# yjxiong/action-detection

Measured on AMD Instinct MI355X. Metric: proposals/sec (9-seg BNInception SSN fwd+bwd), higher is better.
Workload: dtype f32

## Files before the change

### action-detection_amd/_lib.py

```python
import ctypes
import os
import subprocess
import threading

import torch

_HERE = os.path.dirname(os.path.abspath(__file__))
CSRC = os.path.join(_HERE, "csrc")
LIB_PATH = os.path.join(_HERE, "libssn_hip.so")
SOURCES = ["conv_igemm.hip", "conv_x6.hip", "conv_x6_rect.hip", "conv_wgrad.hip", "conv_wgrad_x6.hip", "elementwise.hip", "bn_train.hip", "frames.hip", "detect.hip", "pool.hip", "stpp.hip", "heads_losses.hip", "conv_pl.hip", "planes_ops.hip", "planes_bn.hip", "wgrad_pl.hip", "tag.hip", "eval.hip", "actionness.hip", "train_step.hip", "flow.hip"]

STPP_MAX_PARTS = 24


class SsnStppTable(ctypes.Structure):
    _fields_ = [("n_parts", ctypes.c_int), ("n_seg", ctypes.c_int),
                ("act_lo", ctypes.c_int), ("act_hi", ctypes.c_int),
                ("lo", ctypes.c_int * STPP_MAX_PARTS), ("hi", ctypes.c_int * STPP_MAX_PARTS),
                ("norm", ctypes.c_int * STPP_MAX_PARTS), ("col", ctypes.c_int * STPP_MAX_PARTS)]


_SIGS = {
    "ssn_conv_bn_relu_fwd": "pppppiiiiliiiliiiiipp",
    "ssn_bn_fold": "pppppfppip",
# ... 179 lines not shown
        for name, sig in _SIGS.items():
            fn = getattr(self.cdll, name)
            fn.restype = ctypes.c_int
            fn.argtypes = [_CT[c] for c in sig]
            self._fn[name] = fn

    def call(self, name, *args):
        rc = self._fn[name](*args)
        if rc != 0:
            raise RuntimeError("%s failed (%d): %s" % (name, rc, self.cdll.ssn_last_error().decode()))

    def wgrad_workspace_bytes(self, n, cin, cout, ho, wo, ksize, tile_cfg=-1):
        return int(self.cdll.ssn_conv_wgrad_workspace_bytes(n, cin, cout, ho, wo, ksize, tile_cfg))


_lock = threading.Lock()
_lib = None
_test_lib = None


def _source_stamp(deps, flags):
    import hashlib
    h = hashlib.sha256(" ".join(flags).encode())
    for d in deps:
        h.update(os.path.basename(d).encode())
        with open(d, "rb") as f:
            h.update(f.read())
    return h.hexdigest()


def build(force=False, verbose=False):
    import fcntl
    srcs = [os.path.join(CSRC, s) for s in SOURCES]
    deps = srcs + [os.path.join(CSRC, h) for h in ("ssn_common.h", "conv_epilogue.h", "conv_x6_kernel.h", "planes.h", "conv_pl_epilogue.inc")]
    flags = ["--offload-arch=gfx950", "-O3", "-std=c++17", "-fPIC"]
    stamp_path = LIB_PATH + ".stamp"
    want = _source_stamp(deps, flags)

    def fresh():
        if not os.path.exists(LIB_PATH) or not os.path.exists(stamp_path):
            return False
        with open(stamp_path) as f:
            return f.read().strip() == want

    if not force and fresh():
        return LIB_PATH
    with open(LIB_PATH + ".lock", "w") as lock:
        fcntl.flock(lock, fcntl.LOCK_EX)
        try:
            if not force and fresh():
                return LIB_PATH
            hipcc = os.environ.get("HIPCC", "/opt/rocm/bin/hipcc")
            objs = []
            procs = []
            headers = deps[len(srcs):]
            for s in srcs:
                o = os.path.join(CSRC, os.path.basename(s) + ".o")
                objs.append(o)
                ostamp = _source_stamp([s] + headers, flags)
                try:
                    with open(o + ".stamp") as f:
                        if not force and os.path.exists(o) and f.read().strip() == ostamp:
                            continue
                except OSError:
                    pass
                cmd = [hipcc] + flags + ["-c", s, "-o", o]
                procs.append((cmd, o, ostamp, subprocess.Popen(cmd, stdout=subprocess.PIPE, stderr=subprocess.STDOUT)))
# ... 41 lines not shown
```

### action-detection_amd/csrc/conv_wgrad.hip

```cpp
#include <type_traits>

#include "ssn_common.h"

namespace {

struct WgradArgs {
    const float* g;
    const float* x;
    float* part;
    int N, Cin, H, W;
    long x_img_stride;
    int M, Ho, Wo;
    long g_img_stride;
    int K;
    int ldp;
    int P;
    int pad;
    int splits, chunks_per_split;
    int n_mtiles, n_ktiles;
    uint32_t g_bytes, x_bytes;
    FastDiv div_hw, div_w, div_tiles, div_kt;
};

constexpr int BP = 32;
constexpr int PITCH = 36;
constexpr uint32_t OOB = 0x80000000u;

__device__ __forceinline__ __amdgpu_buffer_rsrc_t make_rsrc(const void* base, uint32_t bytes) {
    return __builtin_amdgcn_make_buffer_rsrc(const_cast<void*>(base), 0, (int)bytes, 0x00020000);
}

template <int KS, int S, int WM, int WN, int TM, int TN>
__global__ __launch_bounds__(256) void conv_wgrad_kernel(WgradArgs p) {
    constexpr int BM = WM * TM * 32;
    constexpr int BN = WN * TN * 32;
// ... 147 lines not shown
#pragma unroll
                    for (int j = 0; j < TN; ++j)
                        acc[i][j] = __builtin_amdgcn_mfma_f32_32x32x2f32(af[cur][i][s], bf[cur][j][s], acc[i][j], 0, 0, 0);
        }
        if (t + 1 < nch) store_slab(buf ^ 1);
        __syncthreads();
    }

    float* out = p.part + (long)z * p.M * p.ldp;
#pragma unroll
    for (int j = 0; j < TN; ++j) {
        const int kk = kk0 + (wn * TN + j) * 32 + li;
        if (kk >= p.K) continue;
#pragma unroll
        for (int i = 0; i < TM; ++i) {
#pragma unroll
            for (int r = 0; r < 16; ++r) {
                const int m = m0 + (wm * TM + i) * 32 + (r & 3) + 8 * (r >> 2) + 4 * lh;
                if (m < p.M) out[(long)m * p.ldp + kk] = acc[i][j][r];
            }
        }
    }
    if (do_bias) {
#pragma unroll
        for (int i = 0; i < TM; ++i) {
            const float tot = rowsum[i] + __shfl_xor(rowsum[i], 32, 64);
            const int m = m0 + (wm * TM + i) * 32 + li;
            if (lh == 0 && m < p.M) out[(long)m * p.ldp + p.K] = tot;
        }
    }
}

__global__ __launch_bounds__(256) void wgrad_reduce_kernel(const float* part, float* dw, float* db, int M, int K,
                                                           int ldp, int splits, int taps) {
    const long total = (long)M * ldp;
    for (long idx = (long)blockIdx.x * 256 + threadIdx.x; idx < total; idx += (long)gridDim.x * 256) {
        float s = 0.f;
        int z = 0;
        for (; z + 8 <= splits; z += 8) {
            float v[8];
#pragma unroll
            for (int q = 0; q < 8; ++q) v[q] = part[(long)(z + q) * total + idx];
#pragma unroll
            for (int q = 0; q < 8; ++q) s += v[q];
        }
        for (; z < splits; ++z) s += part[(long)z * total + idx];
        const int m = (int)(idx / ldp);
        const int kk = (int)(idx - (long)m * ldp);
        if (kk < K) {
            int col = kk;
            if (taps > 1) {
                const int cin = K / taps, t = kk / cin;
                col = (kk - t * cin) * taps + t;
            }
            dw[(long)m * K + col] = s;
        } else if (db) {
            db[m] = s;
        }
    }
}

constexpr int RM_MAX = 48;
struct ReduceTable {
    const float* part[RM_MAX];
    float* dw[RM_MAX];
    float* db[RM_MAX];
    int M[RM_MAX], K[RM_MAX], splits[RM_MAX], taps[RM_MAX];
    int blk0[RM_MAX + 1];
    int count;
};
__global__ __launch_bounds__(256) void wgrad_reduce_multi_kernel(ReduceTable t) {
    int ti = 0;
    while (ti + 1 < t.count && (int)blockIdx.x >= t.blk0[ti + 1]) ++ti;
    const float* part = t.part[ti];
    float* dw = t.dw[ti];
    float* db = t.db[ti];
    const int M = t.M[ti], K = t.K[ti], ldp = K + 1, splits = t.splits[ti], taps = t.taps[ti];
    const long total = (long)M * ldp;
    const uint32_t cin_t = (uint32_t)(K / (taps > 0 ? taps : 1));
    const long nb = t.blk0[ti + 1] - t.blk0[ti];
    for (long idx = (long)((int)blockIdx.x - t.blk0[ti]) * 256 + threadIdx.x; idx < total; idx += nb * 256) {
        float s = 0.f;
        int z = 0;
        for (; z + 8 <= splits; z += 8) {
            float v[8];
#pragma unroll
            for (int q = 0; q < 8; ++q) v[q] = part[(long)(z + q) * total + idx];
#pragma unroll
            for (int q = 0; q < 8; ++q) s += v[q];
        }
        for (; z < splits; ++z) s += part[(long)z * total + idx];
        const int m = (int)((uint32_t)idx / (uint32_t)ldp);
        const int kk = (int)((uint32_t)idx - (uint32_t)m * (uint32_t)ldp);
        if (kk < K) {
            int col = kk;
            if (taps > 1) {
                const int tt = (int)((uint32_t)kk / cin_t);
                col = (kk - tt * (int)cin_t) * taps + tt;
            }
            dw[(long)m * K + col] = s;
        } else if (db) {
            db[m] = s;
        }
    }
}

template <int KS, int S, int WM, int WN, int TM, int TN>
int launch_wgrad(WgradArgs& a, hipStream_t stream) {
    constexpr int BM = WM * TM * 32;
    constexpr int BN = WN * TN * 32;
    a.n_mtiles = (a.M + BM - 1) / BM;
    a.n_ktiles = (a.K + BN - 1) / BN;
    const unsigned tiles = (unsigned)a.n_mtiles * (unsigned)a.n_ktiles;
    a.div_tiles = make_fastdiv(tiles);
    a.div_kt = make_fastdiv((uint32_t)a.n_ktiles);
    hipLaunchKernelGGL((conv_wgrad_kernel<KS, S, WM, WN, TM, TN>), dim3(tiles * (unsigned)a.splits), dim3(256), 0,
                       stream, a);
    SSN_CHECK_LAUNCH("conv_wgrad");
    return SSN_OK;
}

const int kWgBM[7] = {64, 32, 128, 64, 96, 64, 128};
const int kWgBN[7] = {64, 128, 128, 128, 128, 128, 64};

template <int KS, int S>
int launch_wgrad_tile(WgradArgs& a, int cfg, hipStream_t stream) {
    switch (cfg) {
        case 0: return launch_wgrad<KS, S, 2, 2, 1, 1>(a, stream);
        case 1: return launch_wgrad<KS, S, 1, 4, 1, 1>(a, stream);
        case 2: return launch_wgrad<KS, S, 2, 2, 2, 2>(a, stream);
        case 3: return launch_wgrad<KS, S, 2, 2, 1, 2>(a, stream);
        case 4: return launch_wgrad<KS, S, 1, 4, 3, 1>(a, stream);
        case 5: return launch_wgrad<KS, S, 1, 4, 2, 1>(a, stream);
        case 6: return launch_wgrad<KS, S, 2, 2, 2, 1>(a, stream);
    }
    ssn_set_error("conv_wgrad: unknown tile config %d", cfg);
    return SSN_ERR_ARG;
}

int pick_wgrad_tile(int M, int K) {
    double best = 1e300;
    int bc = 0;
    for (int c = 0; c < 7; ++c) {
        const double padded = (double)((M + kWgBM[c] - 1) / kWgBM[c]) * kWgBM[c] *
                              (double)((K + kWgBN[c] - 1) / kWgBN[c]) * kWgBN[c];
        const double reuse = (kWgBM[c] * kWgBN[c] >= 128 * 64) ? 1.0 : 1.12;
        if (padded * reuse < best) {
            best = padded * reuse;
            bc = c;
        }
    }
    return bc;
}

const int kWgOcc[7] = {4, 3, 2, 2, 2, 2, 2};

void plan_wgrad(int M, int K, long P, int cfg, int* splits, int* chunks_per_split) {
    const long tiles = (long)((M + kWgBM[cfg] - 1) / kWgBM[cfg]) * ((K + kWgBN[cfg] - 1) / kWgBN[cfg]);
    plan_split_k(tiles, (P + BP - 1) / BP, kWgOcc[cfg], 8, 6, 0.02 + (double)M * K * 1.6e-6, splits, chunks_per_split);
}

}

extern "C" int ssn_wgrad_reduce_taps(const float* part, float* dw, float* db, int M, int K, int splits, int taps,
                                     hipStream_t stream) {
    SSN_CHECK_ARG(part && dw && M > 0 && K > 0 && splits > 0 && taps >= 1 && K % taps == 0, "wgrad reduce: bad arguments");
    const long total = (long)M * (K + 1);
    long blocks = (total + 255) / 256;
    if (blocks > 2048) blocks = 2048;
    hipLaunchKernelGGL(wgrad_reduce_kernel, dim3((unsigned)blocks), dim3(256), 0, stream, part, dw, db, M, K, K + 1,
                       splits, taps);
    SSN_CHECK_LAUNCH("wgrad_reduce");
    return SSN_OK;
}
extern "C" int ssn_wgrad_reduce(const float* part, float* dw, float* db, int M, int K, int splits, hipStream_t stream) {
    return ssn_wgrad_reduce_taps(part, dw, db, M, K, splits, 1, stream);
}
extern "C" int ssn_wgrad_reduce_multi(int count, const float* const* part, float* const* dw, float* const* db, const int* M,
                                      const int* K, const int* splits, const int* taps, hipStream_t stream) {
    SSN_CHECK_ARG(count >= 0 && (count == 0 || (part && dw && db && M && K && splits && taps)), "wgrad reduce multi: bad arguments");
    for (int base = 0; base < count; base += RM_MAX) {
        ReduceTable t;
        t.count = count - base < RM_MAX ? count - base : RM_MAX;
        int blocks = 0;
        for (int i = 0; i < t.count; ++i) {
            const int j = base + i;
            SSN_CHECK_ARG(part[j] && dw[j] && M[j] > 0 && K[j] > 0 && splits[j] > 0 && taps[j] >= 1 && K[j] % taps[j] == 0 &&
                              (long)M[j] * (K[j] + 1) < (1l << 31),
                          "wgrad reduce multi: bad entry %d", j);
            t.part[i] = part[j];
            t.dw[i] = dw[j];
            t.db[i] = db[j];
            t.M[i] = M[j];
            t.K[i] = K[j];
            t.splits[i] = splits[j];
            t.taps[i] = taps[j];
            t.blk0[i] = blocks;
            long nb = ((long)M[j] * (K[j] + 1) + 255) / 256;
            if (nb > 1024) nb = 1024;
            blocks += (int)nb;
        }
        t.blk0[t.count] = blocks;
        hipLaunchKernelGGL(wgrad_reduce_multi_kernel, dim3((unsigned)blocks), dim3(256), 0, stream, t);
    }
    SSN_CHECK_LAUNCH("wgrad_reduce_multi");
    return SSN_OK;
}

extern "C" long ssn_conv_wgrad_workspace_bytes(int N, int Cin, int Cout, int Ho, int Wo, int ksize, int tile_cfg) {
    const int K = Cin * ksize * ksize;
    const int cfg = tile_cfg >= 0 ? tile_cfg : pick_wgrad_tile(Cout, K);
    int splits, cps;
    plan_wgrad(Cout, K, (long)N * Ho * Wo, cfg, &splits, &cps);
    return (long)splits * Cout * (K + 1) * (long)sizeof(float);
}

extern "C" int ssn_conv_wgrad(const float* g, const float* x, float* dw, float* db, int N, int Cin, int H, int W,
                              long x_img_stride, int Cout, int Ho, int Wo, long g_img_stride, int ksize, int stride,
                              int pad, void* workspace, long ws_bytes, int tile_cfg, hipStream_t stream) {
    SSN_CHECK_ARG(g && x && dw && workspace, "conv wgrad: null pointer");
    SSN_CHECK_ARG(ksize == 1 || ksize == 3 || ksize == 7, "conv wgrad: ksize %d unsupported", ksize);
    WgradArgs a;
    a.g = g;
    a.x = x;
    a.part = (float*)workspace;
    a.N = N;
    a.Cin = Cin;
    a.H = H;
    a.W = W;
    a.x_img_stride = x_img_stride;
    a.M = Cout;
    a.Ho = Ho;
    a.Wo = Wo;
// ... 36 lines not shown
```

### action-detection_amd/csrc/wgrad_pl.hip

```cpp
#include "planes.h"

#include <algorithm>
#include <cmath>
#include <cstdlib>
#include <vector>

namespace {

using namespace pl;

struct WgPlArgs {
    const void* g_hi;
    const void* g_lo;
    const void* x_hi;
    const void* x_lo;
    float* part;
    unsigned long long* trace;
    int dbg;
    const float* g_scale;
    const float* x_scale;
    int g_row_split, g_row_gap;
    int N, Cin, H, W;
    int M;
    int Ho, Wo;
    int kh, kw, stride, pad_h, pad_w;
    int K, ldp;
    int P;
    uint32_t g_img_bytes, g_grp_bytes, x_img_bytes, x_grp_bytes;
    uint32_t g_bytes, x_bytes;
    int splits, ksteps_per_split;
    uint32_t magic_wp;
    int n_mtiles, n_ctiles;
    FastDiv div_hw, div_w, div_tiles, div_ct, div_kk;
};


#ifdef PL_ABLATE
// ... 486 lines not shown
            for (int r = 0; r < 16; ++r) {
                const int m = m0 + (wm * TM + i) * 32 + (r & 3) + 8 * (r >> 2) + 4 * lh;
                if (m < p.M) out[(long)m * p.ldp + p.K] = accb[i][r] * ginv;
            }
    }
    trc.end(p);
}

template <int KK, int TM, int TC, int XP, int KG = 1>
__global__ __launch_bounds__(256 * KG, (KG > 1 || KK * TM * TC >= 18 || TM * TC >= 4) ? 1 : 2) void wgrad_pl9_kernel(WgPlArgs p) {
    __shared__ __attribute__((aligned(1024))) unsigned char lds[wgpl9_lds_bytes<TM, TC, XP>()];
    wgrad_pl9_body<KK, TM, TC, XP, KG>(p, blockIdx.x, lds);
}


constexpr int WGG_MAX = 96;
constexpr int WGG_WRITE = 12;
struct WgGroupEntry {
    WgPlArgs a;
    int variant;
    uint32_t nblk;
};
struct WgGroupIndex {
    int count;
    int blk0[WGG_MAX + 1];
};
struct WgGroupChunk {
    WgGroupEntry e[WGG_WRITE];
    int count;
};
__global__ __launch_bounds__(64) void wgrad_group_write_kernel(WgGroupChunk c, WgGroupEntry* table, int first) {
    if ((int)threadIdx.x < c.count) table[first + threadIdx.x] = c.e[threadIdx.x];
}
__device__ __forceinline__ int group_problem_of_block(const WgGroupIndex& ix, int b) {
    int lo = 0, hi = ix.count - 1;
    while (lo < hi) {
        const int mid = (lo + hi + 1) >> 1;
        if (ix.blk0[mid] <= b) lo = mid; else hi = mid - 1;
    }
    return wave_uniform(lo);
}

template <int XP, int KG, int KH = 3, int KW = 3>
__global__ __launch_bounds__(256 * KG, KG > 1 ? 1 : 2) void wgrad_group9_kernel(const WgGroupEntry* __restrict__ table, WgGroupIndex ix) {
    __shared__ __attribute__((aligned(1024))) unsigned char lds[wgpl9_lds_bytes<1, 1, XP>()];
    const int e = group_problem_of_block(ix, (int)blockIdx.x);
    const uint32_t bid = blockIdx.x - (uint32_t)ix.blk0[e];
    const auto* ent = SSN_CONST_PTR(WgGroupEntry, table) + e;
    if (bid >= ent->nblk) return;
    const WgPlArgs p = ent->a;
    wgrad_pl9_body<KH * KW, 1, 1, XP, KG, KH, KW, KH / 2, KW / 2>(p, bid, lds);
}

constexpr int WGG1_LDS = 65536;
static_assert(wgpl_lds_dwords<2, 2, 2, 2>() * 4 <= WGG1_LDS && wgpl_lds_dwords<1, 4, 3, 1>() * 4 <= WGG1_LDS &&
              wgpl_lds_dwords<2, 2, 1, 1>() * 4 <= WGG1_LDS && wgpl9_lds_bytes<1, 1, 4>() <= WGG1_LDS, "group LDS");
__global__ __launch_bounds__(256, 2) void wgrad_group1_kernel(const WgGroupEntry* __restrict__ table, WgGroupIndex ix) {
    __shared__ __attribute__((aligned(1024))) unsigned char lds[WGG1_LDS];
    const int e = group_problem_of_block(ix, (int)blockIdx.x);
    const uint32_t bid = blockIdx.x - (uint32_t)ix.blk0[e];
    const auto* ent = SSN_CONST_PTR(WgGroupEntry, table) + e;
    if (bid >= ent->nblk) return;
    const WgPlArgs p = ent->a;
    switch (wave_uniform(ent->variant)) {
        case 0: wgrad_pl_body<2, 2, 2, 2>(p, bid, reinterpret_cast<uint32_t*>(lds)); break;
        case 1: wgrad_pl_body<1, 4, 3, 1>(p, bid, reinterpret_cast<uint32_t*>(lds)); break;
        case 2: wgrad_pl_body<2, 2, 1, 1>(p, bid, reinterpret_cast<uint32_t*>(lds)); break;
        default: wgrad_pl9_body<1, 1, 1, 4>(p, bid, lds); break;
    }
}

constexpr int STEM_NS = 128;
constexpr int STEM_DA = 256;
constexpr int STEM_EA = 128;
constexpr int STEM_RING = 1024;
constexpr int STEM_MAX_W = 114;
constexpr int STEM_LDS = 2 * (2 * 2 * 8 * 1024) + 2 * STEM_RING * 32;
inline bool stem_layer(int kh, int kw, int stride, int pad_h, int pad_w, int H, int W, int Ho, int Wo) {
    return kh == 4 && kw == 4 && stride == 1 && pad_h == 2 && pad_w == 2 && Ho == H && Wo == W && W <= STEM_MAX_W;
}
__device__ __forceinline__ void wgrad_stem_body(const WgPlArgs& p, const uint32_t bid, unsigned char* lds) {
    constexpr int NS = STEM_NS, KSC = NS / 16, KG = 2, KSG = KSC / KG;
    constexpr int A_BYTES = 2 * 2 * KSC * 1024;
    constexpr int RING_BYTES = STEM_RING * 32;
    constexpr uint32_t RMASK = STEM_RING - 1;
    static_assert(2 * A_BYTES + 2 * RING_BYTES == STEM_LDS, "LDS size");
    static_assert(STEM_DA >= 2 * (STEM_MAX_W + 2) + 2 && STEM_EA >= STEM_MAX_W + 3 && STEM_DA + 2 * NS + STEM_EA <= STEM_RING, "window");
    unsigned char* const xring = lds + 2 * A_BYTES;

    const int tid = threadIdx.x;
    const int lane = tid & 63, wave8 = wave_uniform(tid >> 6);
    const int wave = wave8 & 3, grp = wave8 >> 2;
    const int wm = wave & 1, wc = wave >> 1;
// ... 116 lines not shown
                accb = __builtin_amdgcn_mfma_f32_32x32x16_f16(af[ks & 1][0], ones, accb, 0, 0, 0);
                accb = __builtin_amdgcn_mfma_f32_32x32x16_f16(af[ks & 1][1], ones, accb, 0, 0, 0);
            }
        }
        buf ^= 1;
    }
    SSN_WAIT_VMCNT(0);

    const float inv = 1.f / (*p.g_scale * *p.x_scale);
    float* out = p.part + ((long)z * KG + grp) * p.M * p.ldp;
    const int ci = c0 + (li & 15);
    if (ci < p.Cin) {
#pragma unroll
        for (int i = 0; i < 4; ++i) {
            const int pi = wc * 4 + i;
            const int t = ((pi >> 2) + 2 * (li >> 4)) * 4 + (pi & 3);
#pragma unroll
            for (int r = 0; r < 16; ++r) {
                const int m = m0 + wm * 32 + (r & 3) + 8 * (r >> 2) + 4 * lh;
                if (m < p.M) out[(long)m * p.ldp + t * p.Cin + ci] = acc[i][r] * inv;
            }
        }
    }
    if (do_bias && li == 0) {
        const float ginv = 1.f / *p.g_scale;
#pragma unroll
        for (int r = 0; r < 16; ++r) {
            const int m = m0 + wm * 32 + (r & 3) + 8 * (r >> 2) + 4 * lh;
            if (m < p.M) out[(long)m * p.ldp + p.K] = accb[r] * ginv;
        }
    }
}

__global__ __launch_bounds__(512, 1) void wgrad_group_stem_kernel(const WgGroupEntry* __restrict__ table, WgGroupIndex ix) {
    __shared__ __attribute__((aligned(1024))) unsigned char lds[STEM_LDS];
    const int e = group_problem_of_block(ix, (int)blockIdx.x);
    const uint32_t bid = blockIdx.x - (uint32_t)ix.blk0[e];
    const auto* ent = SSN_CONST_PTR(WgGroupEntry, table) + e;
    if (bid >= ent->nblk) return;
    const WgPlArgs p = ent->a;
    wgrad_stem_body(p, bid, lds);
}

#undef WG_DMA_B128
#undef WG_RD_FRAG

template <int KK, int TM, int TC, int XP, int KG = 1>
int launch_wgpl9(WgPlArgs& a, hipStream_t stream) {
    constexpr int BM = 2 * TM * 32, BC = 2 * TC * 32;
    a.n_mtiles = (a.M + BM - 1) / BM;
    a.n_ctiles = (a.Cin + BC - 1) / BC;
    const unsigned tiles = (unsigned)a.n_mtiles * (unsigned)a.n_ctiles;
    a.div_tiles = make_fastdiv(tiles);
    a.div_ct = make_fastdiv((uint32_t)a.n_ctiles);
    a.magic_wp = 0xFFFFFFFFu / (uint32_t)(a.W + (KK > 1 ? 1 : 0)) + 1u;
    hipLaunchKernelGGL((wgrad_pl9_kernel<KK, TM, TC, XP, KG>), dim3(tiles * (unsigned)a.splits), dim3(256 * KG), 0, stream, a);
    SSN_CHECK_LAUNCH("wgrad_pl9");
    return SSN_OK;
}

constexpr int N9 = 4;
const int k9BM[N9] = {64, 128, 64, 64};
const int k9BC[N9] = {64, 64, 128, 64};
const int k9Occ[N9] = {1, 1, 1, 1};
const int k9KG[N9] = {1, 1, 1, 2};

template <int XP>
int launch_wgpl9_xp(WgPlArgs& a, int cfg, hipStream_t stream) {
    switch (cfg) {
        case 0: return launch_wgpl9<9, 1, 1, XP>(a, stream);
// ... 313 lines not shown
        it.unit_cost = 3.0 * (kG1BM[v] / 32) * (kG1BC[v] / 32) / 4;
        a.div_kk = make_fastdiv((uint32_t)KK);
    }
    a.div_tiles = make_fastdiv((uint32_t)it.tiles);
    return SSN_OK;
}
void plan_group(std::vector<WgGroupItem*>& fam, int slots, double fixed_cost, int min_units, bool even_units) {
    double work = 0;
    for (WgGroupItem* it : fam) work += (double)it->tiles * (double)it->units * it->unit_cost;
    double target = std::sqrt(2.0 * fixed_cost * work / slots);
    if (target < fixed_cost) target = fixed_cost;
    for (WgGroupItem* it : fam) {
        long per = (long)(target / it->unit_cost + 0.5);
        const long floor_units = (it->family >= WGF_1 && it->chunked) ? (min_units + 3) / 4 : min_units;
        if (per < floor_units) per = floor_units;
        if (per > it->units) per = it->units;
        long splits = (it->units + per - 1) / per;
        per = (it->units + splits - 1) / splits;
        if (even_units && !it->chunked && (per & 1)) ++per;
        splits = (it->units + per - 1) / per;
        it->a.splits = (int)splits;
        it->a.ksteps_per_split = (int)per;
    }
}

bool group1_interleave() {
    static const bool on = [] {
        const char* e = std::getenv("SSN_WGRAD_INTERLEAVE");
        return !(e && e[0] == '0');
    }();
    return on;
}

}

extern "C" void ssn_conv_wgrad_pl_debug_trace(unsigned long long* buf) { g_wg_trace = buf; }
extern "C" void ssn_conv_wgrad_pl_debug_flags(int flags) { g_wg_dbg = flags; }

extern "C" int ssn_wgrad_reduce(const float* part, float* dw, float* db, int M, int K, int splits, hipStream_t stream);
extern "C" int ssn_wgrad_reduce_taps(const float* part, float* dw, float* db, int M, int K, int splits, int taps, hipStream_t stream);

extern "C" int ssn_conv_wgrad_pl_tiles(void) { return NCFG; }

extern "C" long ssn_conv_wgrad_pl_workspace_bytes(int N, int Cin, int Cout, int Ho, int Wo, int kh, int kw, int tile_cfg) {
    if (tile_cfg >= 200) {
        int s1, c1;
        plan1(Cout, Cin, (long)N * Ho * Wo, (tile_cfg - 200) < N1 ? tile_cfg - 200 : 0, &s1, &c1);
        return (long)s1 * Cout * ((long)Cin + 1) * (long)sizeof(float);
    }
    if (tile_cfg >= 100 || (tile_cfg < 0 && kh == 3 && kw == 3)) {
        int c9 = tile_cfg >= 100 ? tile_cfg - 100 : pick_tile9(Cout, Cin, Wo);
        if (c9 >= N9 || (xp_for(Wo) > 8 && c9 != 3)) c9 = 0;
        int splits9, cps9;
        plan9(Cout, Cin, (long)N * (Ho + 1) * (Wo + 1), c9, Wo, &splits9, &cps9);
        const long need9 = (long)splits9 * k9KG[c9] * Cout * ((long)Cin * 9 + 1) * (long)sizeof(float);
        if (tile_cfg >= 100) return need9;
        const int cfg1 = fix_cfg(-1, Cout, Cin);
        int s1, k1;
        plan(Cout, Cin, 9, (long)N * Ho * Wo, cfg1, &s1, &k1);
        const long need1 = (long)s1 * Cout * ((long)Cin * 9 + 1) * (long)sizeof(float);
        return need9 > need1 ? need9 : need1;
    }
    const int cfg = fix_cfg(tile_cfg, Cout, Cin);
    int splits, kps;
    plan(Cout, Cin, kh * kw, (long)N * Ho * Wo, cfg, &splits, &kps);
    return (long)splits * Cout * ((long)Cin * kh * kw + 1) * (long)sizeof(float);
// ... 56 lines not shown
        for (int i = 0; i < count; ++i) {
            plan_out[i * 4] = items[(size_t)i].family;
            plan_out[i * 4 + 1] = items[(size_t)i].variant;
            plan_out[i * 4 + 2] = items[(size_t)i].a.splits;
            plan_out[i * 4 + 3] = items[(size_t)i].a.ksteps_per_split;
        }
    return total;
}

extern "C" int ssn_wgrad_reduce_multi(int count, const float* const* part, float* const* dw, float* const* db, const int* M,
                                      const int* K, const int* splits, const int* taps, hipStream_t stream);

extern "C" int ssn_conv_wgrad_pl_group(int count, const void* const* g_hi, const void* const* g_lo, const void* const* x_hi,
                                       const void* const* x_lo, float* const* dw, float* const* db, const int* shape,
                                       const long* groups, const float* const* g_scale, const float* const* x_scale, void* workspace,
                                       long ws_bytes, void* table, long table_bytes, hipStream_t stream) {
    if (count == 0) return SSN_OK;
    SSN_CHECK_ARG(count > 0 && g_hi && g_lo && x_hi && x_lo && dw && db && shape && groups && g_scale && x_scale && workspace && table,
                  "conv wgrad pl group: null pointer");
    for (int i = 0; i < count; ++i) SSN_CHECK_ARG(dw[i], "conv wgrad pl group: problem %d has no dw", i);
    std::vector<WgGroupItem> items;
    long need = 0;
    int rc = plan_group_all(count, shape, groups, g_hi, g_lo, x_hi, x_lo, dw, db, g_scale, x_scale, items, &need);
    if (rc != SSN_OK) return rc;
    if (ws_bytes < need) {
        ssn_set_error("conv wgrad pl group: workspace %ld < %ld bytes", ws_bytes, need);
        return SSN_ERR_WORKSPACE;
    }
    if (table_bytes < ssn_conv_wgrad_pl_group_table_bytes(count)) {
        ssn_set_error("conv wgrad pl group: table %ld < %ld bytes", table_bytes, ssn_conv_wgrad_pl_group_table_bytes(count));
        return SSN_ERR_WORKSPACE;
    }
    WgGroupEntry* dev = static_cast<WgGroupEntry*>(table);
    int first = 0;
    for (int f = 0; f < WGF_COUNT; ++f) {
        std::vector<WgGroupItem*> fam;
        for (WgGroupItem& it : items)
            if (it.family == f) fam.push_back(&it);
        if (fam.empty()) continue;
        std::stable_sort(fam.begin(), fam.end(), [](const WgGroupItem* x, const WgGroupItem* y) {
            return x->a.ksteps_per_split * x->unit_cost > y->a.ksteps_per_split * y->unit_cost;
        });
        if (f == WGF_1 && group1_interleave()) {
            auto bytes_per_mac = [](const WgGroupItem* x) {
                const double s2 = (double)x->a.stride * x->a.stride;
                return ((double)x->a.M + (double)x->a.Cin * s2) / ((double)x->a.M * x->a.Cin * x->a.kh * x->a.kw);
            };
            std::stable_sort(fam.begin(), fam.end(), [&](const WgGroupItem* x, const WgGroupItem* y) { return bytes_per_mac(x) > bytes_per_mac(y); });
            std::vector<WgGroupItem*> dealt;
            for (size_t lo = 0, hi = fam.size(); lo < hi;) {
                dealt.push_back(fam[lo++]);
                if (lo < hi) dealt.push_back(fam[--hi]);
            }
            fam.swap(dealt);
        }
        for (size_t base = 0; base < fam.size(); base += WGG_MAX) {
            const int n = (int)std::min<size_t>(WGG_MAX, fam.size() - base);
            WgGroupIndex ix;
            ix.count = n;
            long blocks = 0;
            for (int c0 = 0; c0 < n; c0 += WGG_WRITE) {
                WgGroupChunk ch;
                ch.count = std::min(WGG_WRITE, n - c0);
                for (int j = 0; j < ch.count; ++j) {
                    WgGroupItem& it = *fam[base + (size_t)(c0 + j)];
                    it.a.part = reinterpret_cast<float*>(static_cast<char*>(workspace) + it.ws_off);
                    ch.e[j].a = it.a;
                    ch.e[j].variant = it.variant;
                    ch.e[j].nblk = (uint32_t)(it.tiles * it.a.splits);
                    ix.blk0[c0 + j] = (int)blocks;
                    blocks += (it.tiles * it.a.splits + 7) / 8 * 8;
                }
                hipLaunchKernelGGL(wgrad_group_write_kernel, dim3(1), dim3(64), 0, stream, ch, dev, first + c0);
            }
            SSN_CHECK_ARG(blocks < (1l << 31), "conv wgrad pl group: too many blocks");
            for (int j = n; j <= WGG_MAX; ++j) ix.blk0[j] = (int)blocks;
            const WgGroupEntry* tab = dev + first;
            switch (f) {
                case WGF_9_XP6: hipLaunchKernelGGL((wgrad_group9_kernel<6, 1>), dim3((unsigned)blocks), dim3(256), 0, stream, tab, ix); break;
                case WGF_9_XP8: hipLaunchKernelGGL((wgrad_group9_kernel<8, 2>), dim3((unsigned)blocks), dim3(512), 0, stream, tab, ix); break;
                case WGF_9_XP12: hipLaunchKernelGGL((wgrad_group9_kernel<12, 2>), dim3((unsigned)blocks), dim3(512), 0, stream, tab, ix); break;
                case WGF_STEM: hipLaunchKernelGGL(wgrad_group_stem_kernel, dim3((unsigned)blocks), dim3(512), 0, stream, tab, ix); break;
                case WGF_7_ROW: hipLaunchKernelGGL((wgrad_group9_kernel<6, 1, 1, 7>), dim3((unsigned)blocks), dim3(256), 0, stream, tab, ix); break;
                case WGF_7_COL: hipLaunchKernelGGL((wgrad_group9_kernel<12, 2, 7, 1>), dim3((unsigned)blocks), dim3(512), 0, stream, tab, ix); break;
                default: hipLaunchKernelGGL(wgrad_group1_kernel, dim3((unsigned)blocks), dim3(256), 0, stream, tab, ix); break;
            }
            first += n;
        }
    }
    SSN_CHECK_LAUNCH("conv_wgrad_pl_group");
    std::vector<const float*> parts((size_t)count);
    std::vector<float*> dws((size_t)count), dbs((size_t)count);
    std::vector<int> Ms((size_t)count), Ks((size_t)count), sp((size_t)count), tp((size_t)count);
    for (int i = 0; i < count; ++i) {
        const WgGroupItem& it = items[(size_t)i];
        parts[(size_t)i] = reinterpret_cast<const float*>(static_cast<char*>(workspace) + it.ws_off);
        dws[(size_t)i] = it.dw;
        dbs[(size_t)i] = it.db;
        Ms[(size_t)i] = it.a.M;
        Ks[(size_t)i] = it.a.K;
        sp[(size_t)i] = it.a.splits * it.kg;
        tp[(size_t)i] = it.taps;
    }
    return ssn_wgrad_reduce_multi(count, parts.data(), dws.data(), dbs.data(), Ms.data(), Ks.data(), sp.data(), tp.data(), stream);
}

extern "C" int ssn_conv_wgrad_pl(const void* g_hi, const void* g_lo, const void* x_hi, const void* x_lo, float* dw, float* db,
                                 int N, int Cin, int H, int W, long x_img_groups, int Cout, int Ho, int Wo, long g_img_groups,
                                 int kh, int kw, int stride, int pad_h, int pad_w, void* workspace, long ws_bytes, int tile_cfg,
                                 const float* g_scale, const float* x_scale, int g_row_split, int g_row_gap,
                                 int* deferred_reduce, hipStream_t stream) {
    SSN_CHECK_ARG(dw && workspace, "conv wgrad pl: null pointer");
    WgPlArgs a;
    const int rcf = fill_wgpl(a, g_hi, g_lo, x_hi, x_lo, N, Cin, H, W, x_img_groups, Cout, Ho, Wo, g_img_groups, kh, kw, stride, pad_h, pad_w,
                              g_scale, x_scale, g_row_split, g_row_gap);
    if (rcf != SSN_OK) return rcf;
    a.part = (float*)workspace;
    if (tile_cfg >= 200) {
        SSN_CHECK_ARG(chunked_1x1_layer(kh, kw, stride, pad_h, pad_w) && tile_cfg - 200 < N1,
                      "conv wgrad pl: the chunked kernel (tile %d) takes 1x1 / stride-1 layers only", tile_cfg);
        const int c1 = tile_cfg - 200;
        plan1(Cout, Cin, a.P, c1, &a.splits, &a.ksteps_per_split);
        const long need1 = (long)a.splits * Cout * a.ldp * (long)sizeof(float);
        if (ws_bytes < need1) {
            ssn_set_error("conv wgrad pl: workspace %ld < %ld bytes", ws_bytes, need1);
            return SSN_ERR_WORKSPACE;
        }
        a.div_hw = make_fastdiv((uint32_t)(H * W));
        a.div_w = make_fastdiv((uint32_t)W);
        const int rc1 = launch_wgpl1_tile(a, c1, stream);
        if (rc1 != SSN_OK) return rc1;
        if (deferred_reduce) {
            deferred_reduce[0] = a.splits;
            deferred_reduce[1] = 1;
            return SSN_OK;
        }
        return ssn_wgrad_reduce(a.part, dw, db, Cout, a.K, a.splits, stream);
// ... 40 lines not shown
```

Before: 2327.

## Fuse split-K wgrad reduction of previous family into next grouped wgrad launch

Reduction blocks for the previous wgrad family's split-K partials now run interleaved inside the next family's grouped wgrad kernel, instead of one trailing reduce-multi launch. Families are reordered so the one with the fewest partial bytes goes last, leaving the smallest reduce at the tail. The reduce kernel itself also gains float4 vectorized nontemporal loads and a shared helper. This hides reduce bandwidth behind compute-heavy wgrad blocks, at the cost of larger kernel arguments and extra per-block index arithmetic and branching.

```diff
diff --git a/action-detection_amd/_lib.py b/action-detection_amd/_lib.py
--- a/action-detection_amd/_lib.py
+++ b/action-detection_amd/_lib.py
@@ -235,7 +235,7 @@
 def build(force=False, verbose=False):
     import fcntl
     srcs = [os.path.join(CSRC, s) for s in SOURCES]
-    deps = srcs + [os.path.join(CSRC, h) for h in ("ssn_common.h", "conv_epilogue.h", "conv_x6_kernel.h", "planes.h", "conv_pl_epilogue.inc")]
+    deps = srcs + [os.path.join(CSRC, h) for h in ("ssn_common.h", "conv_epilogue.h", "conv_x6_kernel.h", "planes.h", "conv_pl_epilogue.inc", "wgrad_reduce.h")]
     flags = ["--offload-arch=gfx950", "-O3", "-std=c++17", "-fPIC"]
     stamp_path = LIB_PATH + ".stamp"
     want = _source_stamp(deps, flags)
diff --git a/action-detection_amd/csrc/conv_wgrad.hip b/action-detection_amd/csrc/conv_wgrad.hip
--- a/action-detection_amd/csrc/conv_wgrad.hip
+++ b/action-detection_amd/csrc/conv_wgrad.hip
@@ -1,6 +1,7 @@
 #include <type_traits>
 
 #include "ssn_common.h"
+#include "wgrad_reduce.h"
 
 namespace {
 
@@ -214,78 +215,13 @@
 }
 
 __global__ __launch_bounds__(256) void wgrad_reduce_kernel(const float* part, float* dw, float* db, int M, int K,
-                                                           int ldp, int splits, int taps) {
-    const long total = (long)M * ldp;
-    for (long idx = (long)blockIdx.x * 256 + threadIdx.x; idx < total; idx += (long)gridDim.x * 256) {
-        float s = 0.f;
-        int z = 0;
-        for (; z + 8 <= splits; z += 8) {
-            float v[8];
-#pragma unroll
-            for (int q = 0; q < 8; ++q) v[q] = part[(long)(z + q) * total + idx];
-#pragma unroll
-            for (int q = 0; q < 8; ++q) s += v[q];
-        }
-        for (; z < splits; ++z) s += part[(long)z * total + idx];
-        const int m = (int)(idx / ldp);
-        const int kk = (int)(idx - (long)m * ldp);
-        if (kk < K) {
-            int col = kk;
-            if (taps > 1) {
-                const int cin = K / taps, t = kk / cin;
-                col = (kk - t * cin) * taps + t;
-            }
-            dw[(long)m * K + col] = s;
-        } else if (db) {
-            db[m] = s;
-        }
-    }
+                                                           int splits, int taps) {
+    wgrad_reduce_tensor(part, dw, db, M, K, splits, taps, (int)blockIdx.x, (int)gridDim.x);
 }
 
 constexpr int RM_MAX = 48;
-struct ReduceTable {
-    const float* part[RM_MAX];
-    float* dw[RM_MAX];
-    float* db[RM_MAX];
-    int M[RM_MAX], K[RM_MAX], splits[RM_MAX], taps[RM_MAX];
-    int blk0[RM_MAX + 1];
-    int count;
-};
-__global__ __launch_bounds__(256) void wgrad_reduce_multi_kernel(ReduceTable t) {
-    int ti = 0;
-    while (ti + 1 < t.count && (int)blockIdx.x >= t.blk0[ti + 1]) ++ti;
-    const float* part = t.part[ti];
-    float* dw = t.dw[ti];
-    float* db = t.db[ti];
-    const int M = t.M[ti], K = t.K[ti], ldp = K + 1, splits = t.splits[ti], taps = t.taps[ti];
-    const long total = (long)M * ldp;
-    const uint32_t cin_t = (uint32_t)(K / (taps > 0 ? taps : 1));
-    const long nb = t.blk0[ti + 1] - t.blk0[ti];
-    for (long idx = (long)((int)blockIdx.x - t.blk0[ti]) * 256 + threadIdx.x; idx < total; idx += nb * 256) {
-        float s = 0.f;
-        int z = 0;
-        for (; z + 8 <= splits; z += 8) {
-            float v[8];
-#pragma unroll
-            for (int q = 0; q < 8; ++q) v[q] = part[(long)(z + q) * total + idx];
-#pragma unroll
-            for (int q = 0; q < 8; ++q) s += v[q];
-        }
-        for (; z < splits; ++z) s += part[(long)z * total + idx];
-        const int m = (int)((uint32_t)idx / (uint32_t)ldp);
-        const int kk = (int)((uint32_t)idx - (uint32_t)m * (uint32_t)ldp);
-        if (kk < K) {
-            int col = kk;
-            if (taps > 1) {
-                const int tt = (int)((uint32_t)kk / cin_t);
-                col = (kk - tt * (int)cin_t) * taps + tt;
-            }
-            dw[(long)m * K + col] = s;
-        } else if (db) {
-            db[m] = s;
-        }
-    }
-}
+using ReduceTable = WgReduceTable<RM_MAX>;
+__global__ __launch_bounds__(256) void wgrad_reduce_multi_kernel(ReduceTable t) { wgrad_reduce_block(t, (int)blockIdx.x); }
 
 template <int KS, int S, int WM, int WN, int TM, int TN>
 int launch_wgrad(WgradArgs& a, hipStream_t stream) {
@@ -348,10 +284,9 @@
                                      hipStream_t stream) {
     SSN_CHECK_ARG(part && dw && M > 0 && K > 0 && splits > 0 && taps >= 1 && K % taps == 0, "wgrad reduce: bad arguments");
     const long total = (long)M * (K + 1);
-    long blocks = (total + 255) / 256;
-    if (blocks > 2048) blocks = 2048;
-    hipLaunchKernelGGL(wgrad_reduce_kernel, dim3((unsigned)blocks), dim3(256), 0, stream, part, dw, db, M, K, K + 1,
-                       splits, taps);
+    SSN_CHECK_ARG(total < (1l << 31), "wgrad reduce: slab of 2^31 elements or more");
+    const int blocks = wgrad_reduce_blocks(total, 256, 2048);
+    hipLaunchKernelGGL(wgrad_reduce_kernel, dim3((unsigned)blocks), dim3(256), 0, stream, part, dw, db, M, K, splits, taps);
     SSN_CHECK_LAUNCH("wgrad_reduce");
     return SSN_OK;
 }
@@ -378,9 +313,7 @@
             t.splits[i] = splits[j];
             t.taps[i] = taps[j];
             t.blk0[i] = blocks;
-            long nb = ((long)M[j] * (K[j] + 1) + 255) / 256;
-            if (nb > 1024) nb = 1024;
-            blocks += (int)nb;
+            blocks += wgrad_reduce_blocks((long)M[j] * (K[j] + 1), 256, 1024);
         }
         t.blk0[t.count] = blocks;
         hipLaunchKernelGGL(wgrad_reduce_multi_kernel, dim3((unsigned)blocks), dim3(256), 0, stream, t);
diff --git a/action-detection_amd/csrc/wgrad_pl.hip b/action-detection_amd/csrc/wgrad_pl.hip
--- a/action-detection_amd/csrc/wgrad_pl.hip
+++ b/action-detection_amd/csrc/wgrad_pl.hip
@@ -1,8 +1,10 @@
 #include "planes.h"
+#include "wgrad_reduce.h"
 
 #include <algorithm>
 #include <cmath>
 #include <cstdlib>
+#include <cstring>
 #include <vector>
 
 namespace {
@@ -555,6 +557,25 @@
 __global__ __launch_bounds__(64) void wgrad_group_write_kernel(WgGroupChunk c, WgGroupEntry* table, int first) {
     if ((int)threadIdx.x < c.count) table[first + threadIdx.x] = c.e[threadIdx.x];
 }
+constexpr int WGR_MAX = 64;
+struct WgRide {
+    WgReduceTable<WGR_MAX> t;
+    int rblocks;
+    int nminor, phase, minor_is_reduce;
+    FastDiv period;
+};
+static_assert(sizeof(WgGroupIndex) + sizeof(WgRide) + sizeof(void*) <= 4096 - 64, "grouped wgrad kernel arguments");
+__device__ __forceinline__ bool ride_block(const WgRide& rd, uint32_t& b) {
+    if (rd.rblocks == 0) return false;
+    const uint32_t g = b >> 3;
+    uint32_t q, r;
+    fd_divmod(g, rd.period, q, r);
+    const bool minor = r == (uint32_t)rd.phase && q < (uint32_t)rd.nminor;
+    uint32_t before = q + (r > (uint32_t)rd.phase ? 1u : 0u);
+    if (before > (uint32_t)rd.nminor) before = (uint32_t)rd.nminor;
+    b = ((minor ? q : g - before) << 3) | (b & 7u);
+    return minor == (rd.minor_is_reduce != 0);
+}
 __device__ __forceinline__ int group_problem_of_block(const WgGroupIndex& ix, int b) {
     int lo = 0, hi = ix.count - 1;
     while (lo < hi) {
@@ -565,10 +586,15 @@
 }
 
 template <int XP, int KG, int KH = 3, int KW = 3>
-__global__ __launch_bounds__(256 * KG, KG > 1 ? 1 : 2) void wgrad_group9_kernel(const WgGroupEntry* __restrict__ table, WgGroupIndex ix) {
+__global__ __launch_bounds__(256 * KG, KG > 1 ? 1 : 2) void wgrad_group9_kernel(const WgGroupEntry* __restrict__ table, WgGroupIndex ix, WgRide rd) {
     __shared__ __attribute__((aligned(1024))) unsigned char lds[wgpl9_lds_bytes<1, 1, XP>()];
-    const int e = group_problem_of_block(ix, (int)blockIdx.x);
-    const uint32_t bid = blockIdx.x - (uint32_t)ix.blk0[e];
+    uint32_t blk = blockIdx.x;
+    if (ride_block(rd, blk)) {
+        wgrad_reduce_block(rd.t, (int)blk);
+        return;
+    }
+    const int e = group_problem_of_block(ix, (int)blk);
+    const uint32_t bid = blk - (uint32_t)ix.blk0[e];
     const auto* ent = SSN_CONST_PTR(WgGroupEntry, table) + e;
     if (bid >= ent->nblk) return;
     const WgPlArgs p = ent->a;
@@ -578,10 +604,15 @@
 constexpr int WGG1_LDS = 65536;
 static_assert(wgpl_lds_dwords<2, 2, 2, 2>() * 4 <= WGG1_LDS && wgpl_lds_dwords<1, 4, 3, 1>() * 4 <= WGG1_LDS &&
               wgpl_lds_dwords<2, 2, 1, 1>() * 4 <= WGG1_LDS && wgpl9_lds_bytes<1, 1, 4>() <= WGG1_LDS, "group LDS");
-__global__ __launch_bounds__(256, 2) void wgrad_group1_kernel(const WgGroupEntry* __restrict__ table, WgGroupIndex ix) {
+__global__ __launch_bounds__(256, 2) void wgrad_group1_kernel(const WgGroupEntry* __restrict__ table, WgGroupIndex ix, WgRide rd) {
     __shared__ __attribute__((aligned(1024))) unsigned char lds[WGG1_LDS];
-    const int e = group_problem_of_block(ix, (int)blockIdx.x);
-    const uint32_t bid = blockIdx.x - (uint32_t)ix.blk0[e];
+    uint32_t blk = blockIdx.x;
+    if (ride_block(rd, blk)) {
+        wgrad_reduce_block(rd.t, (int)blk);
+        return;
+    }
+    const int e = group_problem_of_block(ix, (int)blk);
+    const uint32_t bid = blk - (uint32_t)ix.blk0[e];
     const auto* ent = SSN_CONST_PTR(WgGroupEntry, table) + e;
     if (bid >= ent->nblk) return;
     const WgPlArgs p = ent->a;
@@ -764,10 +795,15 @@
     }
 }
 
-__global__ __launch_bounds__(512, 1) void wgrad_group_stem_kernel(const WgGroupEntry* __restrict__ table, WgGroupIndex ix) {
+__global__ __launch_bounds__(512, 1) void wgrad_group_stem_kernel(const WgGroupEntry* __restrict__ table, WgGroupIndex ix, WgRide rd) {
     __shared__ __attribute__((aligned(1024))) unsigned char lds[STEM_LDS];
-    const int e = group_problem_of_block(ix, (int)blockIdx.x);
-    const uint32_t bid = blockIdx.x - (uint32_t)ix.blk0[e];
+    uint32_t blk = blockIdx.x;
+    if (ride_block(rd, blk)) {
+        wgrad_reduce_block(rd.t, (int)blk);
+        return;
+    }
+    const int e = group_problem_of_block(ix, (int)blk);
+    const uint32_t bid = blk - (uint32_t)ix.blk0[e];
     const auto* ent = SSN_CONST_PTR(WgGroupEntry, table) + e;
     if (bid >= ent->nblk) return;
     const WgPlArgs p = ent->a;
@@ -1147,6 +1183,16 @@
     return on;
 }
 
+bool wgrad_ride_reduce() {
+    const char* e = std::getenv("SSN_WGRAD_REDUCE");
+    return !(e && std::strcmp(e, "separate") == 0);
+}
+long wgrad_ride_bytes() {
+    const char* e = std::getenv("SSN_WGRAD_RIDE_KB");
+    const long kb = e ? std::atol(e) : 0;
+    return (kb > 0 ? kb : 1536) * 1024;
+}
+
 }
 
 extern "C" void ssn_conv_wgrad_pl_debug_trace(unsigned long long* buf) { g_wg_trace = buf; }
@@ -1269,12 +1315,31 @@
         return SSN_ERR_WORKSPACE;
     }
     WgGroupEntry* dev = static_cast<WgGroupEntry*>(table);
+    std::vector<WgGroupItem*> fams[WGF_COUNT];
+    std::vector<int> order;
+    for (WgGroupItem& it : items) fams[it.family].push_back(&it);
+    {
+        int last = -1;
+        double last_bytes = 0;
+        for (int f = 0; f < WGF_COUNT; ++f) {
+            if (fams[f].empty()) continue;
+            order.push_back(f);
+            double bytes = 0;
+            for (const WgGroupItem* it : fams[f]) bytes += (double)it->a.splits * it->kg * it->a.M * it->a.ldp * 4.0;
+            if (last < 0 || bytes <= last_bytes) {
+                last = f;
+                last_bytes = bytes;
+            }
+        }
+        order.erase(std::find(order.begin(), order.end(), last));
+        order.push_back(last);
+    }
+    const bool ride = wgrad_ride_reduce() && !g_wg_trace;
+    const long ride_bytes = wgrad_ride_bytes();
+    std::vector<const WgGroupItem*> pending, trailing;
     int first = 0;
-    for (int f = 0; f < WGF_COUNT; ++f) {
-        std::vector<WgGroupItem*> fam;
-        for (WgGroupItem& it : items)
-            if (it.family == f) fam.push_back(&it);
-        if (fam.empty()) continue;
+    for (int f : order) {
+        std::vector<WgGroupItem*>& fam = fams[f];
         std::stable_sort(fam.begin(), fam.end(), [](const WgGroupItem* x, const WgGroupItem* y) {
             return x->a.ksteps_per_split * x->unit_cost > y->a.ksteps_per_split * y->unit_cost;
         });
@@ -1310,36 +1375,71 @@
                 }
                 hipLaunchKernelGGL(wgrad_group_write_kernel, dim3(1), dim3(64), 0, stream, ch, dev, first + c0);
             }
-            SSN_CHECK_ARG(blocks < (1l << 31), "conv wgrad pl group: too many blocks");
             for (int j = n; j <= WGG_MAX; ++j) ix.blk0[j] = (int)blocks;
+            WgRide rd;
+            rd.t.count = 0;
+            long rblocks = 0;
+            for (const WgGroupItem* it : pending) {
+                if (!ride || rd.t.count == WGR_MAX) {
+                    trailing.push_back(it);
+                    continue;
+                }
+                const int i = rd.t.count++;
+                const long total = (long)it->a.M * it->a.ldp;
+                SSN_CHECK_ARG(total < (1l << 31), "conv wgrad pl group: slab of 2^31 elements or more");
+                rd.t.part[i] = reinterpret_cast<const float*>(static_cast<char*>(workspace) + it->ws_off);
+                rd.t.dw[i] = it->dw;
+                rd.t.db[i] = it->db;
+                rd.t.M[i] = it->a.M;
+                rd.t.K[i] = it->a.K;
+                rd.t.splits[i] = it->a.splits * it->kg;
+                rd.t.taps[i] = it->taps;
+                rd.t.blk0[i] = (int)rblocks;
+                const long want = (total * 4 * rd.t.splits[i] + ride_bytes - 1) / ride_bytes;
+                rblocks += wgrad_reduce_blocks(total, 256, (int)std::min<long>(want, 1 << 20));
+            }
+            for (int i = rd.t.count; i <= WGR_MAX; ++i) rd.t.blk0[i] = (int)rblocks;
+            pending.clear();
+            const long gm = blocks / 8, gr = (rblocks + 7) / 8;
+            rd.rblocks = (int)rblocks;
+            rd.minor_is_reduce = gr <= gm;
+            rd.nminor = (int)std::min(gm, gr);
+            const long period = rd.nminor > 0 ? (gm + gr) / rd.nminor : 1;
+            rd.phase = (int)(period / 2);
+            rd.period = make_fastdiv((uint32_t)period);
+            const long grid = (gm + gr) * 8;
+            SSN_CHECK_ARG(grid < (1l << 31), "conv wgrad pl group: too many blocks");
             const WgGroupEntry* tab = dev + first;
             switch (f) {
-                case WGF_9_XP6: hipLaunchKernelGGL((wgrad_group9_kernel<6, 1>), dim3((unsigned)blocks), dim3(256), 0, stream, tab, ix); break;
-                case WGF_9_XP8: hipLaunchKernelGGL((wgrad_group9_kernel<8, 2>), dim3((unsigned)blocks), dim3(512), 0, stream, tab, ix); break;
-                case WGF_9_XP12: hipLaunchKernelGGL((wgrad_group9_kernel<12, 2>), dim3((unsigned)blocks), dim3(512), 0, stream, tab, ix); break;
-                case WGF_STEM: hipLaunchKernelGGL(wgrad_group_stem_kernel, dim3((unsigned)blocks), dim3(512), 0, stream, tab, ix); break;
-                case WGF_7_ROW: hipLaunchKernelGGL((wgrad_group9_kernel<6, 1, 1, 7>), dim3((unsigned)blocks), dim3(256), 0, stream, tab, ix); break;
-                case WGF_7_COL: hipLaunchKernelGGL((wgrad_group9_kernel<12, 2, 7, 1>), dim3((unsigned)blocks), dim3(512), 0, stream, tab, ix); break;
-                default: hipLaunchKernelGGL(wgrad_group1_kernel, dim3((unsigned)blocks), dim3(256), 0, stream, tab, ix); break;
-            }
+                case WGF_9_XP6: hipLaunchKernelGGL((wgrad_group9_kernel<6, 1>), dim3((unsigned)grid), dim3(256), 0, stream, tab, ix, rd); break;
+                case WGF_9_XP8: hipLaunchKernelGGL((wgrad_group9_kernel<8, 2>), dim3((unsigned)grid), dim3(512), 0, stream, tab, ix, rd); break;
+                case WGF_9_XP12: hipLaunchKernelGGL((wgrad_group9_kernel<12, 2>), dim3((unsigned)grid), dim3(512), 0, stream, tab, ix, rd); break;
+                case WGF_STEM: hipLaunchKernelGGL(wgrad_group_stem_kernel, dim3((unsigned)grid), dim3(512), 0, stream, tab, ix, rd); break;
+                case WGF_7_ROW: hipLaunchKernelGGL((wgrad_group9_kernel<6, 1, 1, 7>), dim3((unsigned)grid), dim3(256), 0, stream, tab, ix, rd); break;
+                case WGF_7_COL: hipLaunchKernelGGL((wgrad_group9_kernel<12, 2, 7, 1>), dim3((unsigned)grid), dim3(512), 0, stream, tab, ix, rd); break;
+                default: hipLaunchKernelGGL(wgrad_group1_kernel, dim3((unsigned)grid), dim3(256), 0, stream, tab, ix, rd); break;
+            }
+            for (int j = 0; j < n; ++j) pending.push_back(fam[base + (size_t)j]);
             first += n;
         }
     }
     SSN_CHECK_LAUNCH("conv_wgrad_pl_group");
-    std::vector<const float*> parts((size_t)count);
-    std::vector<float*> dws((size_t)count), dbs((size_t)count);
-    std::vector<int> Ms((size_t)count), Ks((size_t)count), sp((size_t)count), tp((size_t)count);
-    for (int i = 0; i < count; ++i) {
-        const WgGroupItem& it = items[(size_t)i];
-        parts[(size_t)i] = reinterpret_cast<const float*>(static_cast<char*>(workspace) + it.ws_off);
-        dws[(size_t)i] = it.dw;
-        dbs[(size_t)i] = it.db;
-        Ms[(size_t)i] = it.a.M;
-        Ks[(size_t)i] = it.a.K;
-        sp[(size_t)i] = it.a.splits * it.kg;
-        tp[(size_t)i] = it.taps;
-    }
-    return ssn_wgrad_reduce_multi(count, parts.data(), dws.data(), dbs.data(), Ms.data(), Ks.data(), sp.data(), tp.data(), stream);
+    trailing.insert(trailing.end(), pending.begin(), pending.end());
+    const size_t nt = trailing.size();
+    std::vector<const float*> parts(nt);
+    std::vector<float*> dws(nt), dbs(nt);
+    std::vector<int> Ms(nt), Ks(nt), sp(nt), tp(nt);
+    for (size_t i = 0; i < nt; ++i) {
+        const WgGroupItem& it = *trailing[i];
+        parts[i] = reinterpret_cast<const float*>(static_cast<char*>(workspace) + it.ws_off);
+        dws[i] = it.dw;
+        dbs[i] = it.db;
+        Ms[i] = it.a.M;
+        Ks[i] = it.a.K;
+        sp[i] = it.a.splits * it.kg;
+        tp[i] = it.taps;
+    }
+    return ssn_wgrad_reduce_multi((int)nt, parts.data(), dws.data(), dbs.data(), Ms.data(), Ks.data(), sp.data(), tp.data(), stream);
 }
 
 extern "C" int ssn_conv_wgrad_pl(const void* g_hi, const void* g_lo, const void* x_hi, const void* x_lo, float* dw, float* db,
diff --git a/action-detection_amd/csrc/wgrad_reduce.h b/action-detection_amd/csrc/wgrad_reduce.h
--- /dev/null
+++ b/action-detection_amd/csrc/wgrad_reduce.h
@@ -0,0 +1,92 @@
+#pragma once
+#include "ssn_common.h"
+
+typedef float wgr_f32x4 __attribute__((ext_vector_type(4)));
+
+template <int N>
+struct WgReduceTable {
+    const float* part[N];
+    float* dw[N];
+    float* db[N];
+    int M[N], K[N], splits[N], taps[N];
+    int blk0[N + 1];
+    int count;
+};
+
+__device__ __forceinline__ void wgrad_reduce_put(float s, int m, int kk, float* dw, float* db, int K, int taps, uint32_t cin_t) {
+    if (kk < K) {
+        int col = kk;
+        if (taps > 1) {
+            const int tt = (int)((uint32_t)kk / cin_t);
+            col = (kk - tt * (int)cin_t) * taps + tt;
+        }
+        dw[(long)m * K + col] = s;
+    } else if (db) {
+        db[m] = s;
+    }
+}
+
+__device__ __forceinline__ void wgrad_reduce_tensor(const float* part, float* dw, float* db, int M, int K, int splits, int taps, int blk, int nb) {
+    const int ldp = K + 1;
+    const long total = (long)M * ldp;
+    const uint32_t cin_t = (uint32_t)(K / (taps > 0 ? taps : 1));
+    const long nt = (long)blockDim.x;
+    if ((total & 3) == 0 && (reinterpret_cast<uintptr_t>(part) & 15) == 0) {
+        for (long idx = ((long)blk * nt + threadIdx.x) * 4; idx < total; idx += (long)nb * nt * 4) {
+            wgr_f32x4 s = {0.f, 0.f, 0.f, 0.f};
+            int z = 0;
+            for (; z + 8 <= splits; z += 8) {
+                wgr_f32x4 v[8];
+#pragma unroll
+                for (int q = 0; q < 8; ++q) v[q] = __builtin_nontemporal_load(reinterpret_cast<const wgr_f32x4*>(part + (long)(z + q) * total + idx));
+#pragma unroll
+                for (int q = 0; q < 8; ++q) s += v[q];
+            }
+            for (; z < splits; ++z) s += __builtin_nontemporal_load(reinterpret_cast<const wgr_f32x4*>(part + (long)z * total + idx));
+            int m = (int)((uint32_t)idx / (uint32_t)ldp);
+            int kk = (int)((uint32_t)idx - (uint32_t)m * (uint32_t)ldp);
+#pragma unroll
+            for (int q = 0; q < 4; ++q) {
+                wgrad_reduce_put(s[q], m, kk, dw, db, K, taps, cin_t);
+                if (++kk == ldp) {
+                    kk = 0;
+                    ++m;
+                }
+            }
+        }
+        return;
+    }
+    for (long idx = (long)blk * nt + threadIdx.x; idx < total; idx += (long)nb * nt) {
+        float s = 0.f;
+        int z = 0;
+        for (; z + 8 <= splits; z += 8) {
+            float v[8];
+#pragma unroll
+            for (int q = 0; q < 8; ++q) v[q] = __builtin_nontemporal_load(part + (long)(z + q) * total + idx);
+#pragma unroll
+            for (int q = 0; q < 8; ++q) s += v[q];
+        }
+        for (; z < splits; ++z) s += __builtin_nontemporal_load(part + (long)z * total + idx);
+        const int m = (int)((uint32_t)idx / (uint32_t)ldp);
+        wgrad_reduce_put(s, m, (int)((uint32_t)idx - (uint32_t)m * (uint32_t)ldp), dw, db, K, taps, cin_t);
+    }
+}
+
+template <int N>
+__device__ __forceinline__ void wgrad_reduce_block(const WgReduceTable<N>& t, int b) {
+    if (b >= t.blk0[t.count]) return;
+    int lo = 0, hi = t.count - 1;
+    while (lo < hi) {
+        const int mid = (lo + hi + 1) >> 1;
+        if (t.blk0[mid] <= b) lo = mid; else hi = mid - 1;
+    }
+    const int ti = wave_uniform(lo);
+    wgrad_reduce_tensor(t.part[ti], t.dw[ti], t.db[ti], t.M[ti], t.K[ti], t.splits[ti], t.taps[ti], b - t.blk0[ti], t.blk0[ti + 1] - t.blk0[ti]);
+}
+
+static inline int wgrad_reduce_blocks(long total, int threads, int cap) {
+    const long per = (long)threads * ((total & 3) == 0 ? 4 : 1);
+    long nb = (total + per - 1) / per;
+    if (nb > cap) nb = cap;
+    return (int)(nb < 1 ? 1 : nb);
+}
```

Result: no change. 2321 (-0.3%).
